# koadman/libMems

Measured on AMD Instinct MI355X. Metric: seed-mers/sec sorted+matched (+ MUMs/sec) at 1/2/4/8 MI355X; HBM GB/s vs roofline, higher is better.
Workload: dtype u64; 1 GPU; BASELINE config 3: 8 x 100 Mbp, seed weight 19 (0x7b974ef), MemHash seed stage (sorted+matched); genomes=8, genome_length=100000000, seedmers_total=799999792, seedmers_rank0=799999792, probes_rank0=100459493, parallelism=1 GPU

## Files before the change

include/mums.h:

```cpp
#ifndef MUMS_H
#define MUMS_H

#include <stdint.h>

#ifdef __cplusplus
extern "C" {
#endif

#define MUMS_ABI_VERSION 6

enum mums_status {
    MUMS_OK = 0,
    MUMS_E_INVALID = -1,
    MUMS_E_NOMEM = -2,
    MUMS_E_HIP = -3,
    MUMS_E_GAP = -4,
    MUMS_E_UNSUPPORTED = -5,
    MUMS_E_NODEVICE = -6
};

enum mums_stage {
    MUMS_STAGE_SEEDS = 1,
    MUMS_STAGE_ALL = 2
};
// ... 40 lines not shown

int  mums_set_seed(mums_ctx* ctx, uint64_t pattern);
int  mums_set_params(mums_ctx* ctx, uint32_t repeat_tol, uint32_t enum_tol, uint32_t table_size);
int  mums_set_mask(mums_ctx* ctx, int masked, uint64_t seq_mask);
int  mums_set_parallel_compat(mums_ctx* ctx, int enable, uint64_t chunk_size);
int  mums_set_pairwise(mums_ctx* ctx, int enable);

int  mums_add_genome(mums_ctx* ctx, const char* ascii, uint64_t n);
int  mums_add_genome_device(mums_ctx* ctx, const void* d_ascii, uint64_t n);
int  mums_genome_device(mums_ctx* ctx, uint32_t genome, const void** d_ascii, uint64_t* n);
int  mums_clear(mums_ctx* ctx);
int  mums_clear_sequences(mums_ctx* ctx);

int  mums_set_start_points(mums_ctx* ctx, const uint64_t* start_points, uint32_t count);
int  mums_get_offset_log(mums_ctx* ctx, uint64_t* out, uint64_t cap_rows, uint64_t* rows, uint32_t* seq_count);
int  mums_find(mums_ctx* ctx);
int  mums_find_stage(mums_ctx* ctx, int stage);

int  mums_result_count(mums_ctx* ctx, uint64_t* count, uint32_t* seq_count);
int  mums_result_copy(mums_ctx* ctx, uint64_t* lengths, int64_t* starts);

int  mums_mem_table_count(mums_ctx* ctx, uint32_t* counts, uint32_t table_size);
int  mums_get_stats(mums_ctx* ctx, mums_stats* out);
int  mums_set_profiling(mums_ctx* ctx, int enable);
const char* mums_last_error(mums_ctx* ctx);

int64_t  mums_get_seed(int weight, int seed_rank);
uint32_t mums_default_seed_weight(uint64_t avg_len);
int  mums_copy_seed_keys(mums_ctx* ctx, uint32_t genome, uint64_t* out, uint64_t cap);
int  mums_copy_seed_keys_range(mums_ctx* ctx, uint32_t genome, uint64_t first, uint64_t count, uint64_t* out);
int  mums_build_sml(mums_ctx* ctx, uint32_t genome, uint32_t* positions, uint64_t cap);
int  mums_seed_occurrence(mums_ctx* ctx, uint32_t genome, float* freq, uint64_t cap);
int  mums_multiplicity_filter(mums_ctx* ctx, uint32_t multiplicity);
int  mums_write_sml(mums_ctx* ctx, uint32_t genome, const char* path, const char* description);
int  mums_add_genome_sml(mums_ctx* ctx, const char* path, uint64_t* seed_out);
int  mums_length_filter(mums_ctx* ctx, uint64_t min_length);
int  mums_set_match_log(mums_ctx* ctx, int enable);
int  mums_match_log_copy(mums_ctx* ctx, uint64_t* lengths, int64_t* starts, uint64_t capacity, uint64_t* count);
int  mums_set_progress_log(mums_ctx* ctx, int enable);
int  mums_progress_log_copy(mums_ctx* ctx, char* text, uint64_t capacity, uint64_t* length);
int  mums_eliminate_overlaps(mums_ctx* ctx);
int  mums_eliminate_overlaps_v2(mums_ctx* ctx, const uint32_t* seq_ids, uint32_t count, int eliminate_both);
int  mums_load_matches(mums_ctx* ctx, uint32_t seq_count, uint64_t count, const uint64_t* lengths,
                       const int64_t* starts);
int  mums_find_batch(mums_ctx* ctx, uint32_t B, uint32_t G, const char* ascii, const uint64_t* seq_off);
int  mums_batch_info(mums_ctx* ctx, uint64_t* match_off, uint64_t* probes, uint64_t* collisions, uint64_t* restarts);
int  mums_anchor_batch(mums_ctx* ctx, uint32_t B, uint32_t G, const char* ascii, const uint64_t* seq_off,
                       const uint64_t* patterns, uint32_t rounds, int eliminate_both, uint64_t min_length);
int  mums_anchor_tail_batch(mums_ctx* ctx, uint32_t B, uint32_t G, const uint64_t* match_off,
                            const uint64_t* lengths, const int64_t* starts, int eliminate_both, uint64_t min_length);
int  mums_anchor_batch_info(mums_ctx* ctx, uint64_t* match_off, uint64_t* table_entries, uint64_t* probes,
                            uint64_t* collisions, uint64_t* restarts);
int  mums_debug_std_sort(mums_ctx* ctx, const uint64_t* keys, uint64_t n, int depth_override, uint32_t* ids);

int  mums_shard_layout(mums_ctx* ctx, uint32_t genomes_total, uint32_t first_genome, const uint64_t* lengths);
int  mums_shard_slice(mums_ctx* ctx, uint32_t genomes_total, const uint64_t* lengths, uint32_t genome,
                      uint64_t pos_begin, uint64_t pos_end);
int  mums_shard_msd_bits(mums_ctx* ctx, uint32_t* msd_bits, uint64_t* local_records);
int  mums_shard_keys(mums_ctx* ctx, uint64_t* d_records, uint64_t capacity, uint64_t* bucket_counts);
int  mums_shard_merge(mums_ctx* ctx, const uint64_t* d_records, uint32_t nsources, uint32_t first_bucket,
                      uint32_t nbuckets, const uint64_t* counts);
int  mums_shard_restart_pending(mums_ctx* ctx, uint64_t* pending);
int  mums_shard_stream(mums_ctx* ctx, const void** d_records, uint64_t* n);
int  mums_shard_restart_plan(mums_ctx* ctx, uint64_t* d_stream, uint32_t nranks, const uint64_t* counts,
                             const uint32_t* first_bucket, const uint32_t* nbuckets, void* d_out,
                             uint64_t capacity_bytes, uint64_t* block_bytes);
int  mums_shard_restart_apply(mums_ctx* ctx, const void* d_block, uint64_t restarts, const uint64_t* offset_log);
int  mums_shard_restart_counts(mums_ctx* ctx, uint64_t* info);
int  mums_shard_restart_prepare(mums_ctx* ctx, uint32_t nranks, uint32_t rank, const uint64_t* all_info,
                                uint64_t* S0);
int  mums_shard_restart_step(mums_ctx* ctx, uint64_t* S, uint64_t* restarts, uint64_t* undecidable);
int  mums_shard_restart_log(mums_ctx* ctx, uint64_t* rkey, uint64_t* rS);
int  mums_shard_restart_runs(mums_ctx* ctx, uint64_t restarts, const uint64_t* rkey, const uint64_t* rS,
                             uint64_t* runs, uint64_t capacity, uint64_t* nruns);
int  mums_shard_restart_ties(mums_ctx* ctx, const uint32_t* d_packed_all, const uint64_t* runs, uint64_t nruns,
                             const uint64_t* vofs, uint32_t* d_out);
int  mums_shard_restart_finish(mums_ctx* ctx, uint64_t restarts, const uint64_t* rkey, const uint64_t* rS,
                               const uint64_t* runs, uint64_t nruns, const uint32_t* d_pos, const uint64_t* vofs);
int  mums_shard_restart_info(mums_ctx* ctx, uint64_t* info);
int  mums_shard_tie_flags(mums_ctx* ctx, const uint64_t* gofs, uint32_t* d_out);
int  mums_shard_tie_replay(mums_ctx* ctx, const uint32_t* d_packed_all, uint32_t genome, uint32_t nparts,
                           const uint32_t* d_flags, const uint64_t* flag_off, const uint64_t* lens, uint32_t* d_out,
                           const uint64_t* out_off);
int  mums_shard_tie_apply(mums_ctx* ctx, const uint32_t* d_ids, const uint64_t* vofs);
int  mums_probe_count(mums_ctx* ctx, uint64_t* count);
int  mums_shard_bucket_counts(mums_ctx* ctx, uint64_t* counts);
int  mums_shard_probe_rows(mums_ctx* ctx, uint32_t nranks, const uint32_t* bounds, int64_t* d_rows,
                           uint64_t capacity_rows, uint64_t* counts);
int  mums_shard_packed_info(mums_ctx* ctx, uint64_t* word_offset, uint64_t* nwords, uint64_t* total_words);
int  mums_shard_packed_copy(mums_ctx* ctx, uint32_t* d_dst);
int  mums_shard_find(mums_ctx* ctx, const int64_t* d_rows, uint64_t nrows, const uint32_t* d_packed_all);
int  mums_shard_chain_label(mums_ctx* ctx, const uint32_t* d_packed_all, uint64_t* nchains);
int  mums_shard_chain_export(mums_ctx* ctx, uint32_t nranks, const uint32_t* bounds, int64_t* d_rows, uint32_t* d_tags,
                             uint64_t capacity_rows, int64_t* d_entries, uint32_t* d_first, uint64_t capacity_entries,
                             uint64_t* row_counts, uint64_t* entry_counts);
int  mums_shard_find_labelled(mums_ctx* ctx, const int64_t* d_rows, const uint32_t* d_tags, uint64_t nrows,
                              const int64_t* d_entries, const uint32_t* d_first, uint64_t nentries, uint32_t nsrc,
                              const uint64_t* src_rows, const uint64_t* src_entries, const uint32_t* d_packed_all);
int  mums_shard_chain_info(mums_ctx* ctx, uint64_t* info);
int  mums_shard_chain_entries(mums_ctx* ctx, uint32_t nranks, const uint32_t* bounds, int64_t* d_entries,
                              uint64_t capacity_entries, uint64_t* entry_counts);
int  mums_shard_entry_thresholds(mums_ctx* ctx, const int64_t* d_entries, uint64_t nentries, uint32_t* d_thr);
int  mums_shard_kept_export(mums_ctx* ctx, uint32_t nranks, const uint32_t* d_thr, int64_t* d_rows, uint32_t* d_tags,
                            uint64_t capacity_rows, uint32_t* d_first, uint64_t* row_counts, uint64_t* dropped_counts);
int  mums_shard_find_kept(mums_ctx* ctx, const int64_t* d_rows, const uint32_t* d_tags, uint64_t nrows,
                          const int64_t* d_entries, const uint32_t* d_first, uint64_t nentries, uint32_t nsrc,
// ... 29 lines not shown
```

libmems_amd/__init__.py:

```python
from __future__ import annotations

import ctypes
import os
from dataclasses import dataclass
from typing import List, Optional, Sequence

import numpy as np

_HERE = os.path.dirname(os.path.abspath(__file__))
LIB_PATH = os.environ.get("MUMS_DEV_LIB") or os.path.join(_HERE, "libmums_hip.so")

MUMS_OK = 0
MUMS_E_INVALID = -1
MUMS_E_NOMEM = -2
MUMS_E_HIP = -3
MUMS_E_GAP = -4
MUMS_E_UNSUPPORTED = -5
MUMS_E_NODEVICE = -6

STAGE_SEEDS = 1
STAGE_ALL = 2

DEFAULT_MEM_TABLE_SIZE = 40000
DEFAULT_REPEAT_TOLERANCE = 0
# ... 20 lines not shown
        ("mem_count", ctypes.c_uint64),
        ("collision_count", ctypes.c_uint64),
        ("repeat_limit_groups", ctypes.c_uint64),
        ("nonempty_buckets", ctypes.c_uint64),
        ("ms_keys", ctypes.c_double),
        ("ms_sort", ctypes.c_double),
        ("ms_groups", ctypes.c_double),
        ("ms_buckets", ctypes.c_double),
        ("ms_replay", ctypes.c_double),
        ("ms_output", ctypes.c_double),
        ("ms_total", ctypes.c_double),
        ("ms_dominant", ctypes.c_double),
        ("dominant_launches", ctypes.c_uint64),
        ("dominant_bytes", ctypes.c_uint64),
        ("key_bytes", ctypes.c_uint64),
        ("sort_passes", ctypes.c_uint64),
        ("ms_chains", ctypes.c_double),
        ("chains", ctypes.c_uint64),
        ("chunks", ctypes.c_uint64),
        ("restarts", ctypes.c_uint64),
        ("ms_chain_walks", ctypes.c_double),
        ("chain_walk_words", ctypes.c_uint64),
        ("chain_walks", ctypes.c_uint64),
        ("chain_walk_bytes", ctypes.c_uint64),
        ("ms_short_walks", ctypes.c_double),
        ("short_walk_words", ctypes.c_uint64),
        ("short_walks", ctypes.c_uint64),
        ("short_walk_bytes", ctypes.c_uint64),
    ]


EXPORTED_SYMBOLS = [
    "mums_abi_version", "mums_ctx_create", "mums_ctx_destroy", "mums_set_stream", "mums_set_seed",
    "mums_set_params", "mums_set_mask", "mums_add_genome", "mums_add_genome_device", "mums_clear",
    "mums_find", "mums_find_stage", "mums_result_count", "mums_result_copy", "mums_get_stats",
    "mums_last_error", "mums_get_seed", "mums_default_seed_weight", "mums_copy_seed_keys",
    "mums_build_sml", "mums_set_profiling", "mums_shard_layout", "mums_shard_msd_bits", "mums_shard_keys",
    "mums_shard_merge", "mums_probe_count", "mums_probe_copy", "mums_shard_bucket_counts", "mums_shard_probe_rows",
    "mums_shard_packed_info", "mums_shard_packed_copy", "mums_shard_find", "mums_set_parallel_compat",
    "mums_seed_occurrence", "mums_multiplicity_filter", "mums_length_filter", "mums_write_sml",
    "mums_add_genome_sml", "mums_set_pairwise", "mums_shard_slice", "mums_set_start_points",
    "mums_get_offset_log", "mums_copy_seed_keys_range", "mums_mem_table_count", "mums_eliminate_overlaps",
    "mums_load_matches", "mums_debug_std_sort", "mums_comm_unique_id", "mums_comm_init_rank", "mums_comm_init_all",
    "mums_comm_init_local", "mums_comm_destroy", "mums_comm_last_error", "mums_shard_key_ranges", "mums_shard_run",
    "mums_set_match_log", "mums_match_log_copy", "mums_shard_restart_pending", "mums_shard_stream",
    "mums_shard_restart_plan", "mums_shard_restart_apply", "mums_comm_init_host", "mums_set_progress_log",
    "mums_progress_log_copy", "mums_shard_restart_counts", "mums_shard_restart_prepare", "mums_shard_restart_step",
    "mums_shard_restart_log", "mums_shard_restart_runs", "mums_shard_restart_ties", "mums_shard_restart_finish",
    "mums_shard_restart_info", "mums_shard_tie_flags", "mums_shard_tie_replay", "mums_shard_tie_apply",
    "mums_genome_device", "mums_shard_chain_label", "mums_shard_chain_export", "mums_shard_find_labelled",
    "mums_shard_chain_info", "mums_shard_chain_entries", "mums_shard_entry_thresholds", "mums_shard_kept_export",
    "mums_shard_find_kept", "mums_comm_exchange_info", "mums_eliminate_overlaps_v2", "mums_clear_sequences",
    "mums_find_batch", "mums_batch_info", "mums_anchor_batch", "mums_anchor_tail_batch", "mums_anchor_batch_info",
]

COMM_ALLGATHER_FN = ctypes.CFUNCTYPE(ctypes.c_int, ctypes.c_void_p, ctypes.POINTER(ctypes.c_uint64), ctypes.c_uint64,
                                     ctypes.POINTER(ctypes.c_uint64))
COMM_ALLTOALLV_FN = ctypes.CFUNCTYPE(ctypes.c_int, ctypes.c_void_p, ctypes.c_void_p, ctypes.POINTER(ctypes.c_uint64),
                                     ctypes.c_void_p, ctypes.POINTER(ctypes.c_uint64))


class MumsCommOps(ctypes.Structure):
    _fields_ = [("allgather_u64", COMM_ALLGATHER_FN), ("alltoallv", COMM_ALLTOALLV_FN)]

_lib: Optional[ctypes.CDLL] = None


def load_library(path: str = LIB_PATH) -> ctypes.CDLL:
    global _lib
    if _lib is not None:
        return _lib
    if not os.path.exists(path):
        raise ImportError(f"{path} not built: run `make -C {_HERE}` (hipcc --offload-arch=gfx950)")
    try:
        import torch
    except ImportError:
        pass
    lib = ctypes.CDLL(path)
    vp, u64, u32, i32 = ctypes.c_void_p, ctypes.c_uint64, ctypes.c_uint32, ctypes.c_int
    lib.mums_abi_version.restype = i32
    lib.mums_ctx_create.argtypes = [i32, ctypes.POINTER(vp)]
    lib.mums_ctx_destroy.argtypes = [vp]
    lib.mums_set_stream.argtypes = [vp, vp]
    lib.mums_set_seed.argtypes = [vp, u64]
    lib.mums_set_params.argtypes = [vp, u32, u32, u32]
    lib.mums_set_mask.argtypes = [vp, i32, u64]
    lib.mums_add_genome.argtypes = [vp, ctypes.c_char_p, u64]
    lib.mums_add_genome_device.argtypes = [vp, vp, u64]
    lib.mums_genome_device.argtypes = [vp, u32, ctypes.POINTER(vp), ctypes.POINTER(u64)]
    lib.mums_shard_chain_label.argtypes = [vp, vp, vp]
    lib.mums_shard_chain_export.argtypes = [vp, u32, vp, vp, vp, u64, vp, vp, u64, vp, vp]
    lib.mums_shard_find_labelled.argtypes = [vp, vp, vp, u64, vp, vp, u64, u32, vp, vp, vp]
    lib.mums_shard_chain_info.argtypes = [vp, vp]
    lib.mums_shard_chain_entries.argtypes = [vp, u32, vp, vp, u64, vp]
    lib.mums_shard_entry_thresholds.argtypes = [vp, vp, u64, vp]
    lib.mums_shard_kept_export.argtypes = [vp, u32, vp, vp, vp, u64, vp, vp, vp]
    lib.mums_shard_find_kept.argtypes = [vp, vp, vp, u64, vp, vp, u64, u32, vp, vp, u64, vp]
    lib.mums_comm_exchange_info.argtypes = [vp, vp]
    lib.mums_clear.argtypes = [vp]
    lib.mums_clear_sequences.argtypes = [vp]
    lib.mums_find.argtypes = [vp]
    lib.mums_find_stage.argtypes = [vp, i32]
    lib.mums_result_count.argtypes = [vp, ctypes.POINTER(u64), ctypes.POINTER(u32)]
    lib.mums_result_copy.argtypes = [vp, vp, vp]
    lib.mums_get_stats.argtypes = [vp, ctypes.POINTER(_Stats)]
    lib.mums_last_error.argtypes = [vp]
    lib.mums_last_error.restype = ctypes.c_char_p
    lib.mums_get_seed.argtypes = [i32, i32]
    lib.mums_get_seed.restype = ctypes.c_int64
    lib.mums_default_seed_weight.argtypes = [u64]
    lib.mums_default_seed_weight.restype = u32
    lib.mums_copy_seed_keys.argtypes = [vp, u32, vp, u64]
    lib.mums_build_sml.argtypes = [vp, u32, vp, u64]
    lib.mums_set_profiling.argtypes = [vp, i32]
    lib.mums_shard_layout.argtypes = [vp, u32, u32, vp]
    lib.mums_shard_msd_bits.argtypes = [vp, ctypes.POINTER(u32), ctypes.POINTER(u64)]
    lib.mums_shard_keys.argtypes = [vp, vp, u64, vp]
    lib.mums_shard_merge.argtypes = [vp, vp, u32, u32, u32, vp]
    lib.mums_probe_count.argtypes = [vp, ctypes.POINTER(u64)]
    lib.mums_probe_copy.argtypes = [vp, vp, vp, u64]
    lib.mums_shard_bucket_counts.argtypes = [vp, vp]
    lib.mums_shard_probe_rows.argtypes = [vp, u32, vp, vp, u64, vp]
    lib.mums_shard_packed_info.argtypes = [vp, ctypes.POINTER(u64), ctypes.POINTER(u64), ctypes.POINTER(u64)]
    lib.mums_shard_packed_copy.argtypes = [vp, vp]
    lib.mums_shard_find.argtypes = [vp, vp, u64, vp]
    lib.mums_set_parallel_compat.argtypes = [vp, i32, u64]
    lib.mums_seed_occurrence.argtypes = [vp, u32, vp, u64]
    lib.mums_multiplicity_filter.argtypes = [vp, u32]
    lib.mums_length_filter.argtypes = [vp, u64]
    lib.mums_write_sml.argtypes = [vp, u32, ctypes.c_char_p, ctypes.c_char_p]
    lib.mums_add_genome_sml.argtypes = [vp, ctypes.c_char_p, ctypes.POINTER(u64)]
    lib.mums_set_pairwise.argtypes = [vp, i32]
    lib.mums_shard_slice.argtypes = [vp, u32, vp, u32, u64, u64]
    lib.mums_set_start_points.argtypes = [vp, vp, u32]
    lib.mums_copy_seed_keys_range.argtypes = [vp, u32, u64, u64, vp]
    lib.mums_mem_table_count.argtypes = [vp, vp, u32]
    lib.mums_get_offset_log.argtypes = [vp, vp, u64, ctypes.POINTER(u64), ctypes.POINTER(u32)]
    lib.mums_eliminate_overlaps.argtypes = [vp]
    lib.mums_eliminate_overlaps_v2.argtypes = [vp, vp, u32, ctypes.c_int]
    lib.mums_load_matches.argtypes = [vp, u32, u64, vp, vp]
    lib.mums_debug_std_sort.argtypes = [vp, vp, u64, ctypes.c_int, vp]
    lib.mums_comm_unique_id.argtypes = [vp, u64]
    lib.mums_comm_init_rank.argtypes = [ctypes.POINTER(vp), ctypes.c_int, ctypes.c_int, ctypes.c_int, vp]
    lib.mums_comm_init_all.argtypes = [ctypes.POINTER(vp), ctypes.c_int, vp]
    lib.mums_comm_init_local.argtypes = [ctypes.POINTER(vp), ctypes.c_int, vp]
    lib.mums_comm_init_host.argtypes = [ctypes.POINTER(vp), ctypes.c_int, ctypes.c_int, ctypes.c_int,
                                        ctypes.POINTER(MumsCommOps), vp]
    lib.mums_comm_destroy.argtypes = [vp]
    lib.mums_comm_destroy.restype = None
    lib.mums_comm_last_error.argtypes = [vp]
    lib.mums_comm_last_error.restype = ctypes.c_char_p
    lib.mums_shard_key_ranges.argtypes = [vp, u32, u32, vp, vp]
    lib.mums_shard_run.argtypes = [vp, vp, ctypes.c_int]
    lib.mums_shard_restart_pending.argtypes = [vp, vp]
    lib.mums_shard_stream.argtypes = [vp, vp, vp]
    lib.mums_shard_restart_plan.argtypes = [vp, vp, u32, vp, vp, vp, vp, u64, vp]
    lib.mums_shard_restart_apply.argtypes = [vp, vp, u64, vp]
    lib.mums_shard_restart_counts.argtypes = [vp, vp]
    lib.mums_shard_restart_prepare.argtypes = [vp, u32, u32, vp, vp]
    lib.mums_shard_restart_step.argtypes = [vp, vp, vp, vp]
    lib.mums_shard_restart_log.argtypes = [vp, vp, vp]
    lib.mums_shard_restart_runs.argtypes = [vp, u64, vp, vp, vp, u64, vp]
    lib.mums_shard_restart_ties.argtypes = [vp, vp, vp, u64, vp, vp]
    lib.mums_shard_restart_finish.argtypes = [vp, u64, vp, vp, vp, u64, vp, vp]
    lib.mums_shard_restart_info.argtypes = [vp, vp]
    lib.mums_shard_tie_flags.argtypes = [vp, vp, vp]
    lib.mums_shard_tie_replay.argtypes = [vp, vp, u32, u32, vp, vp, vp, vp, vp]
    lib.mums_shard_tie_apply.argtypes = [vp, vp, vp]
    lib.mums_set_match_log.argtypes = [vp, i32]
    lib.mums_set_progress_log.argtypes = [vp, i32]
    lib.mums_progress_log_copy.argtypes = [vp, ctypes.c_char_p, u64, ctypes.POINTER(u64)]
    lib.mums_match_log_copy.argtypes = [vp, vp, vp, u64, ctypes.POINTER(u64)]
    lib.mums_find_batch.argtypes = [vp, u32, u32, vp, vp]
    lib.mums_batch_info.argtypes = [vp, vp, vp, vp, vp]
    lib.mums_anchor_batch.argtypes = [vp, u32, u32, vp, vp, vp, u32, i32, u64]
    lib.mums_anchor_tail_batch.argtypes = [vp, u32, u32, vp, vp, vp, i32, u64]
    lib.mums_anchor_batch_info.argtypes = [vp, vp, vp, vp, vp, vp]
    _lib = lib
    return lib


def getSeed(weight: int, seed_rank: int = 0) -> int:
    return int(load_library().mums_get_seed(weight, seed_rank)) & 0xFFFFFFFFFFFFFFFF


def getSeedLength(seed: int) -> int:
    if seed == 0:
        return 0
    s = seed & 0xFFFFFFFFFFFFFFFF
    lo = (s & -s).bit_length() - 1
    return s.bit_length() - lo


def getSeedWeight(seed: int) -> int:
# ... 384 lines not shown

    def SetMatchLog(self, enable: bool = True) -> None:
        self._check(self._lib.mums_set_match_log(self._ctx, int(bool(enable))))

    def MatchLog(self) -> "MatchList":
        n = ctypes.c_uint64()
        self._check(self._lib.mums_match_log_copy(self._ctx, None, None, 0, ctypes.byref(n)))
        g = ctypes.c_uint32()
        cnt = ctypes.c_uint64()
        self._check(self._lib.mums_result_count(self._ctx, ctypes.byref(cnt), ctypes.byref(g)))
        lengths = np.zeros(n.value, dtype=np.uint64)
        starts = np.zeros((n.value, g.value), dtype=np.int64)
        if n.value:
            self._check(self._lib.mums_match_log_copy(self._ctx, lengths.ctypes.data, starts.ctypes.data, n.value,
                                                      ctypes.byref(n)))
        return MatchList(lengths, starts)

    def LogProgress(self, enable: bool = True) -> None:
        self._check(self._lib.mums_set_progress_log(self._ctx, int(bool(enable))))

    def ProgressLog(self) -> str:
        n = ctypes.c_uint64()
        self._check(self._lib.mums_progress_log_copy(self._ctx, None, 0, ctypes.byref(n)))
        buf = ctypes.create_string_buffer(n.value + 1)
        self._check(self._lib.mums_progress_log_copy(self._ctx, buf, n.value + 1, ctypes.byref(n)))
        return buf.value.decode()

    def EliminateOverlaps(self) -> None:
        self._check(self._lib.mums_eliminate_overlaps(self._ctx))

    def EliminateOverlaps_v2(self, seq_ids=None, eliminate_both: bool = False) -> None:
        if seq_ids is None:
            self._check(self._lib.mums_eliminate_overlaps_v2(self._ctx, None, 0, int(bool(eliminate_both))))
            return
        for i in seq_ids:
            if not 0 <= int(i) < 2 ** 32:
                raise MumsError(MUMS_E_INVALID, f"EliminateOverlaps_v2: sequence id {i} out of range")
        n = len(seq_ids)
        ids = np.zeros(max(n, 1), dtype=np.uint32)
        ids[:n] = [int(i) for i in seq_ids]
        self._check(self._lib.mums_eliminate_overlaps_v2(self._ctx, ids.ctypes.data, n, int(bool(eliminate_both))))

    def LoadMatches(self, ml: "MatchList") -> None:
        lengths = np.ascontiguousarray(ml.lengths, dtype=np.uint64)
        starts = np.ascontiguousarray(ml.starts, dtype=np.int64)
        M, G = starts.shape
        self._check(self._lib.mums_load_matches(self._ctx, G, M, lengths.ctypes.data, starts.ctypes.data))

    def _debug_std_sort(self, keys: np.ndarray, depth: int = -1) -> np.ndarray:
        keys = np.ascontiguousarray(keys, dtype=np.uint64)
        ids = np.zeros(len(keys), dtype=np.uint32)
        self._check(self._lib.mums_debug_std_sort(self._ctx, keys.ctypes.data, len(keys), depth, ids.ctypes.data))
        return ids


def shard_key_ranges(totals, world: int):
    lib = load_library()
    t = np.ascontiguousarray(totals, dtype=np.uint64)
    f = np.zeros(world, dtype=np.uint32)
    c = np.zeros(world, dtype=np.uint32)
    rc = lib.mums_shard_key_ranges(t.ctypes.data, len(t), world, f.ctypes.data, c.ctypes.data)
    if rc != MUMS_OK:
        raise MumsError(rc, "mums_shard_key_ranges")
    return [(int(a), int(b)) for a, b in zip(f, c)]


class ShardedMemHash:

    def __init__(self, devices: Sequence[int], comm: str = "rccl", table_size: int = 40000, layout: str = "blocks",
                 parallel_compat: bool = False, chunk_size: int = 200000, pairwise: bool = False):
        if layout not in ("blocks", "slices"):
            raise ValueError("layout: 'blocks' or 'slices'")
        self.layout = layout
        self.parallel_compat = bool(parallel_compat)
        self.pairwise = bool(pairwise)
        self.chunk_size = int(chunk_size)
        self._lib = load_library()
        self.devices = list(devices)
        self.world = len(self.devices)
        self.comm_kind = comm
        self.table_size = table_size
        self.seed = 0
        self.repeat_tol = 0
        self.enum_tol = 1
        self.progress = False
        self.match_log = False
        self.seqs: List[bytes] = []
        self.ranks: List[MemHash] = []
        self.stats_per_rank: List[dict] = []
        self.rank_status: List[int] = []
        comms = (ctypes.c_void_p * self.world)()
        devs = (ctypes.c_int * self.world)(*self.devices)
        init = self._lib.mums_comm_init_all if comm == "rccl" else self._lib.mums_comm_init_local
        rc = init(comms, self.world, devs)
        if rc != MUMS_OK:
            raise MumsError(rc, f"mums_comm_init ({comm}) failed")
        self._comms = [comms[r] for r in range(self.world)]

    def SetSeed(self, seed: int) -> None:
        self.seed = seed

    def SetRepeatTolerance(self, t: int) -> None:
        self.repeat_tol = int(t)

    def SetEnumerationTolerance(self, t: int) -> None:
        self.enum_tol = int(t)
# ... 189 lines not shown
```

libmems_amd/csrc/mums_capi.hip:

```cpp
#include <hip/hip_runtime.h>

#include <algorithm>
#include <array>
#include <chrono>
#include <functional>
#include <cstddef>
#include <cstdio>
#include <cstdlib>
#include <cstring>
#include <memory>
#include <string>
#include <vector>

#include "../../include/mums.h"
#include "match_device.h"
#include "mums_internal.h"
#include "seed_device.h"

using namespace mums;

namespace {

struct DevBuf {
    void* p = nullptr;
// ... 3699 lines not shown
    }
    uint64_t P = 0, C = 0, R = 0, E = 0;
    for (uint32_t p = 0; p < B; ++p) {
        P += ctx->batch_probes[p];
        C += ctx->batch_coll[p];
        R += ctx->batch_restarts[p];
        E += ctx->anchor_table[p];
    }
    mums_stats& s = ctx->st;
    s = mums_stats{};
    s.seedmers = Nstat;
    s.probes = P;
    s.mem_count = E;
    s.collision_count = C;
    s.restarts = R;
    s.repeat_limit_groups = R;
    s.key_bytes = 8;
    for (const Round& x : rd) s.sort_passes += (uint64_t)((x.kbits + pbits + 7) / 8);
    s.ms_keys = ms_keys;
    s.ms_sort = ms_sort;
    s.ms_replay = ms_replay;
    s.ms_output = anchor_ms(ctx, EV_REPLAY, EV_OUTPUT);
    s.ms_total = anchor_ms(ctx, EV_START, EV_OUTPUT);
    return anchor_done(ctx, G, M, P, Nstat);
}

int mums_anchor_batch_info(mums_ctx* ctx, uint64_t* match_off, uint64_t* table_entries, uint64_t* probes,
                           uint64_t* collisions, uint64_t* restarts) {
    if (check_ctx(ctx)) return MUMS_E_INVALID;
    if (!ctx->batch_result || !ctx->anchor_result)
        return fail(ctx, MUMS_E_INVALID, "no completed mums_anchor_batch / mums_anchor_tail_batch on this context");
    if (match_off) std::copy(ctx->batch_off.begin(), ctx->batch_off.end(), match_off);
    if (table_entries) std::copy(ctx->anchor_table.begin(), ctx->anchor_table.end(), table_entries);
    if (probes) std::copy(ctx->batch_probes.begin(), ctx->batch_probes.end(), probes);
    if (collisions) std::copy(ctx->batch_coll.begin(), ctx->batch_coll.end(), collisions);
    if (restarts) std::copy(ctx->batch_restarts.begin(), ctx->batch_restarts.end(), restarts);
    return MUMS_OK;
}

int mums_debug_std_sort(mums_ctx* ctx, const uint64_t* keys, uint64_t n, int depth_override, uint32_t* ids) {
    if (check_ctx(ctx) || (n && (!keys || !ids))) return MUMS_E_INVALID;
    if (n >= 0xFFFFFFF0ull) return fail(ctx, MUMS_E_UNSUPPORTED, "n >= 2^32");
    if (n == 0) return MUMS_OK;
    HIPCHK(hipSetDevice(ctx->device));
    HIPCHK(ctx->flen.ensure(n * 8 + 8));
    HIPCHK(ctx->fs.ensure(n * 4 + 8));
    HIPCHK(h2d_sync(ctx->flen.p, keys, n * 8, ctx->stream));
    HIPCHK(eo_sort_ids(ctx->eo, ctx->flen.as<uint64_t>(), (uint32_t)n, depth_override, ctx->fs.as<uint32_t>(),
                       ctx->stream));
    HIPCHK(hipMemcpy(ids, ctx->fs.p, n * 4, hipMemcpyDeviceToHost));
    return MUMS_OK;
}


int mums_shard_layout(mums_ctx* ctx, uint32_t genomes_total, uint32_t first_genome, const uint64_t* lengths) {
    if (check_ctx(ctx)) return MUMS_E_INVALID;
    if (genomes_total > (uint32_t)kMaxG) return fail(ctx, MUMS_E_UNSUPPORTED, "more than 64 genomes");
    if (first_genome > genomes_total || (genomes_total && !lengths))
        return fail(ctx, MUMS_E_INVALID, "bad shard layout");
    ctx->shard = true;
    ctx->slice = false;
    ctx->shard_first = first_genome;
    ctx->shard_len.assign(lengths, lengths + genomes_total);
    ctx->stage_done = 0;
    return MUMS_OK;
}

int mums_shard_slice(mums_ctx* ctx, uint32_t genomes_total, const uint64_t* lengths, uint32_t genome,
                     uint64_t pos_begin, uint64_t pos_end) {
    if (check_ctx(ctx)) return MUMS_E_INVALID;
    if (genomes_total > (uint32_t)kMaxG) return fail(ctx, MUMS_E_UNSUPPORTED, "more than 64 genomes");
    if (genome >= genomes_total || !lengths || pos_begin > pos_end) return fail(ctx, MUMS_E_INVALID, "bad slice");
    ctx->shard = true;
    ctx->slice = true;
    ctx->shard_first = genome;
    ctx->slice_genome = genome;
    ctx->slice_begin = pos_begin;
    ctx->slice_end = pos_end;
    ctx->shard_len.assign(lengths, lengths + genomes_total);
    ctx->stage_done = 0;
    return MUMS_OK;
}

int mums_shard_msd_bits(mums_ctx* ctx, uint32_t* msd_bits, uint64_t* local_records) {
    if (check_ctx(ctx)) return MUMS_E_INVALID;
    int rc = prepare_shard(ctx);
    if (rc) return rc;
    if (msd_bits) *msd_bits = (uint32_t)ctx->msd_bits;
    if (local_records) {
        uint64_t n = 0;
        for (int g = 0; g < ctx->lgt.G; ++g) n += ctx->lgt.m[g];
        *local_records = n;
    }
    return MUMS_OK;
}

int mums_shard_keys(mums_ctx* ctx, uint64_t* d_records, uint64_t capacity, uint64_t* bucket_counts) {
    if (check_ctx(ctx)) return MUMS_E_INVALID;
    if (!have_device()) return fail(ctx, MUMS_E_NODEVICE, "no HIP device");
    HIPCHK(hipSetDevice(ctx->device));
    int rc = prepare_shard(ctx);
    if (rc) return rc;
    GenomeTable& l = ctx->lgt;
    uint64_t n = 0;
    for (int g = 0; g < l.G; ++g) n += l.m[g];
    if (n > capacity || (n && !d_records)) return fail(ctx, MUMS_E_INVALID, "record buffer too small");
// ... 2704 lines not shown
```

libmems_amd/csrc/radix_sort.hip:

```cpp
#include <cstdlib>
#include "mums_internal.h"

namespace mums {

namespace {

constexpr int kRTile = 4096;
constexpr int kRounds = kRTile / kBlock;
constexpr int kWaves = kBlock / 64;
constexpr int kDigits = 256;

template <typename K>
__global__ __launch_bounds__(kBlock) void rs_upsweep(const K* __restrict__ keys, uint64_t n, int shift,
                                                     uint32_t* __restrict__ hist, uint32_t nblocks, int agg) {
    __shared__ uint32_t h[kWaves][kDigits];
    const int lane = threadIdx.x & 63, wv = threadIdx.x >> 6;
    for (int i = threadIdx.x; i < kWaves * kDigits; i += kBlock) (&h[0][0])[i] = 0;
    __syncthreads();
    const uint64_t b0 = (uint64_t)blockIdx.x * kRTile + (uint64_t)wv * (kRTile / kWaves);
    if (agg) {
        #pragma unroll 4
        for (int r = 0; r < kRounds; ++r) {
            const uint64_t i = b0 + (uint64_t)r * 64 + lane;
            const bool valid = i < n;
            const uint32_t d = valid ? (uint32_t)(keys[i] >> shift) & 0xFFu : 0u;
            uint32_t tot;
            const uint32_t rk = wave_match_rank<8>(d, valid, &tot);
            if (valid && rk == 0) atomicAdd(&h[wv][d], tot);
        }
    } else {
        #pragma unroll 4
        for (int r = 0; r < kRounds; ++r) {
            uint64_t i = b0 + (uint64_t)r * 64 + lane;
            if (i < n) {
                uint32_t d = (uint32_t)(keys[i] >> shift) & 0xFFu;
                atomicAdd(&h[wv][d], 1u);
            }
        }
    }
    __syncthreads();
    const int t = threadIdx.x;
    uint32_t s = 0;
    #pragma unroll
    for (int w = 0; w < kWaves; ++w) s += h[w][t];
    hist[(uint64_t)t * nblocks + blockIdx.x] = s;
}

template <typename K, bool kImplicitVals>
__global__ __launch_bounds__(kBlock) void rs_downsweep(const K* __restrict__ kin, const uint32_t* __restrict__ vin,
                                                       uint64_t n, int shift, const uint32_t* __restrict__ hist,
                                                       uint32_t nblocks, K* __restrict__ kout,
                                                       uint32_t* __restrict__ vout) {
    __shared__ K skeys[kRTile];
    __shared__ uint32_t svals[kRTile];
    __shared__ uint32_t wcnt[kWaves][kDigits];
    __shared__ uint32_t lstart[kDigits];
    __shared__ uint32_t gofs[kDigits];
    __shared__ uint32_t s_w[kWaves];
    const int lane = threadIdx.x & 63, wv = threadIdx.x >> 6;
    for (int i = threadIdx.x; i < kWaves * kDigits; i += kBlock) (&wcnt[0][0])[i] = 0;
    __syncthreads();

    const uint64_t tile0 = (uint64_t)blockIdx.x * kRTile;
    const uint64_t b0 = tile0 + (uint64_t)wv * (kRTile / kWaves);
    K key[kRounds];
    uint32_t val[kRounds];
    uint32_t rank[kRounds];
    #pragma unroll
    for (int r = 0; r < kRounds; ++r) {
        const uint64_t i = b0 + (uint64_t)r * 64 + lane;
        const bool valid = i < n;
        key[r] = valid ? kin[i] : (K)0;
        val[r] = kImplicitVals ? (uint32_t)i : (valid ? vin[i] : 0u);
        const uint32_t d = (uint32_t)(key[r] >> shift) & 0xFFu;
        uint32_t tot;
        const uint32_t rk = wave_match_rank<8>(d, valid, &tot);
        uint32_t old = 0;
        if (valid) old = wcnt[wv][d];
        if (valid && rk == 0) wcnt[wv][d] = old + tot;
        rank[r] = old + rk;
    }
    __syncthreads();

    {
        const int t = threadIdx.x;
        uint32_t acc = 0;
        #pragma unroll
        for (int w = 0; w < kWaves; ++w) {
            uint32_t c = wcnt[w][t];
            wcnt[w][t] = acc;
            acc += c;
        }
        uint32_t v = acc;
        #pragma unroll
        for (int d = 1; d < 64; d <<= 1) {
            uint32_t x = __shfl_up(v, d, 64);
            if (lane >= d) v += x;
        }
        if (lane == 63) s_w[wv] = v;
        __syncthreads();
        uint32_t wpre = 0;
        #pragma unroll
        for (int w = 0; w < kWaves; ++w) wpre += (w < wv) ? s_w[w] : 0u;
        lstart[t] = wpre + v - acc;
        gofs[t] = hist[(uint64_t)t * nblocks + blockIdx.x];
    }
    __syncthreads();

    #pragma unroll
    for (int r = 0; r < kRounds; ++r) {
        const uint64_t i = b0 + (uint64_t)r * 64 + lane;
        if (i < n) {
            const uint32_t d = (uint32_t)(key[r] >> shift) & 0xFFu;
            const uint32_t lp = lstart[d] + wcnt[wv][d] + rank[r];
            skeys[lp] = key[r];
            svals[lp] = val[r];
        }
    }
    __syncthreads();

    const uint64_t cnt = (n - tile0) < (uint64_t)kRTile ? (n - tile0) : (uint64_t)kRTile;
    #pragma unroll
    for (int r = 0; r < kRounds; ++r) {
        const uint32_t s = threadIdx.x + r * kBlock;
        if (s < cnt) {
            const K k = skeys[s];
            const uint32_t d = (uint32_t)(k >> shift) & 0xFFu;
            const uint64_t o = (uint64_t)gofs[d] + (s - lstart[d]);
            kout[o] = k;
            vout[o] = svals[s];
        }
    }
}

uint64_t tiles(uint64_t n) { return (n + kRTile - 1) / kRTile; }

}

size_t radix_tmp_bytes(uint64_t n) {
    uint64_t h = (uint64_t)kDigits * tiles(n);
    return (h + 64) * sizeof(uint32_t) + scan_tmp_bytes(h) + 256;
}

template <typename K>
hipError_t radix_sort(const K* keys_in, const uint32_t* vals_in, uint64_t n, int bits, K* kA, uint32_t* vA,
                      K* kB, uint32_t* vB, void* d_tmp, int* out_buf, hipStream_t st, hipEvent_t* ev_ds) {
    const int passes = (bits + 7) / 8;
    *out_buf = (passes - 1) % 2;
    if (n == 0 || passes == 0) return hipSuccess;
    const uint32_t nb = (uint32_t)tiles(n);
    uint32_t* hist = (uint32_t*)d_tmp;
    void* stmp = (void*)(hist + (uint64_t)kDigits * nb + 64);
    const K* ksrc = keys_in;
    const uint32_t* vsrc = vals_in;
    for (int p = 0; p < passes; ++p) {
        K* kdst = (p % 2 == 0) ? kA : kB;
        uint32_t* vdst = (p % 2 == 0) ? vA : vB;
        const int shift = 8 * p;
        const bool agg = !getenv("MUMS_DEV_RS_NOAGG");
        hipLaunchKernelGGL(rs_upsweep<K>, dim3(nb), dim3(kBlock), 0, st, ksrc, n, shift, hist, nb, agg ? 1 : 0);
        hipError_t e = exclusive_scan_u32(hist, (uint64_t)kDigits * nb, stmp, nullptr, st);
        if (e != hipSuccess) return e;
        if (ev_ds) (void)hipEventRecord(ev_ds[2 * p], st);
        if (vsrc == nullptr)
            hipLaunchKernelGGL((rs_downsweep<K, true>), dim3(nb), dim3(kBlock), 0, st, ksrc, vsrc, n, shift, hist,
                               nb, kdst, vdst);
        else
            hipLaunchKernelGGL((rs_downsweep<K, false>), dim3(nb), dim3(kBlock), 0, st, ksrc, vsrc, n, shift, hist,
                               nb, kdst, vdst);
        e = hipGetLastError();
        if (e != hipSuccess) return e;
        if (ev_ds) (void)hipEventRecord(ev_ds[2 * p + 1], st);
        ksrc = kdst;
        vsrc = vdst;
    }
    return hipSuccess;
}

template hipError_t radix_sort<uint32_t>(const uint32_t*, const uint32_t*, uint64_t, int, uint32_t*, uint32_t*,
                                         uint32_t*, uint32_t*, void*, int*, hipStream_t, hipEvent_t*);
template hipError_t radix_sort<uint64_t>(const uint64_t*, const uint32_t*, uint64_t, int, uint64_t*, uint32_t*,
                                         uint64_t*, uint32_t*, void*, int*, hipStream_t, hipEvent_t*);

}
```

Before: 40.03 billion seed-mers/s.

## Restructure radix sort upsweep and specialize downsweep on digit width

Rewrites the radix upsweep so that each wave counts a whole 4096-key tile using vectorized 16-byte loads and ballot-based digit aggregation. Each block now covers several tiles and writes the histograms out in coalesced order. The downsweep is templated on the actual digit bit-width of the last pass and runs with 512 threads, using 16-bit per-wave counters. These changes target memory throughput and shared-memory atomic cost in the sort. They add complexity and more template instantiations, and the uint16 counters could overflow if the tile size grows. A debug entry point for timing the radix sort is also added.

```diff
diff --git a/include/mums.h b/include/mums.h
--- a/include/mums.h
+++ b/include/mums.h
@@ -116,6 +116,8 @@
 int  mums_anchor_batch_info(mums_ctx* ctx, uint64_t* match_off, uint64_t* table_entries, uint64_t* probes,
                             uint64_t* collisions, uint64_t* restarts);
 int  mums_debug_std_sort(mums_ctx* ctx, const uint64_t* keys, uint64_t n, int depth_override, uint32_t* ids);
+int  mums_debug_radix_sort(mums_ctx* ctx, const void* d_keys, int key_bytes, uint64_t n, int bits,
+                           void* d_keys_out, uint32_t* d_ids_out, float* ms);
 
 int  mums_shard_layout(mums_ctx* ctx, uint32_t genomes_total, uint32_t first_genome, const uint64_t* lengths);
 int  mums_shard_slice(mums_ctx* ctx, uint32_t genomes_total, const uint64_t* lengths, uint32_t genome,
diff --git a/libmems_amd/__init__.py b/libmems_amd/__init__.py
--- a/libmems_amd/__init__.py
+++ b/libmems_amd/__init__.py
@@ -96,6 +96,7 @@
     "mums_shard_chain_info", "mums_shard_chain_entries", "mums_shard_entry_thresholds", "mums_shard_kept_export",
     "mums_shard_find_kept", "mums_comm_exchange_info", "mums_eliminate_overlaps_v2", "mums_clear_sequences",
     "mums_find_batch", "mums_batch_info", "mums_anchor_batch", "mums_anchor_tail_batch", "mums_anchor_batch_info",
+    "mums_debug_radix_sort",
 ]
 
 COMM_ALLGATHER_FN = ctypes.CFUNCTYPE(ctypes.c_int, ctypes.c_void_p, ctypes.POINTER(ctypes.c_uint64), ctypes.c_uint64,
@@ -184,6 +185,7 @@
     lib.mums_eliminate_overlaps_v2.argtypes = [vp, vp, u32, ctypes.c_int]
     lib.mums_load_matches.argtypes = [vp, u32, u64, vp, vp]
     lib.mums_debug_std_sort.argtypes = [vp, vp, u64, ctypes.c_int, vp]
+    lib.mums_debug_radix_sort.argtypes = [vp, vp, i32, u64, i32, vp, vp, ctypes.POINTER(ctypes.c_float)]
     lib.mums_comm_unique_id.argtypes = [vp, u64]
     lib.mums_comm_init_rank.argtypes = [ctypes.POINTER(vp), ctypes.c_int, ctypes.c_int, ctypes.c_int, vp]
     lib.mums_comm_init_all.argtypes = [ctypes.POINTER(vp), ctypes.c_int, vp]
@@ -674,6 +676,20 @@
         ids = np.zeros(len(keys), dtype=np.uint32)
         self._check(self._lib.mums_debug_std_sort(self._ctx, keys.ctypes.data, len(keys), depth, ids.ctypes.data))
         return ids
+
+    def _debug_radix_sort(self, keys, bits: int):
+        import torch
+
+        if keys.dim() != 1 or not keys.is_cuda or not keys.is_contiguous() or keys.element_size() not in (4, 8):
+            raise MumsError(MUMS_E_INVALID, "_debug_radix_sort: a contiguous 1-D device tensor of 4-B or 8-B keys")
+        n = keys.numel()
+        kout = torch.empty_like(keys)
+        ids = torch.empty(n, dtype=torch.int32, device=keys.device)
+        ms = ctypes.c_float(0.0)
+        torch.cuda.synchronize(keys.device)
+        self._check(self._lib.mums_debug_radix_sort(self._ctx, keys.data_ptr(), keys.element_size(), n, int(bits),
+                                                    kout.data_ptr(), ids.data_ptr(), ctypes.byref(ms)))
+        return kout, ids, float(ms.value)
 
 
 def shard_key_ranges(totals, world: int):
diff --git a/libmems_amd/csrc/mums_capi.hip b/libmems_amd/csrc/mums_capi.hip
--- a/libmems_amd/csrc/mums_capi.hip
+++ b/libmems_amd/csrc/mums_capi.hip
@@ -3775,6 +3775,49 @@
     return MUMS_OK;
 }
 
+int mums_debug_radix_sort(mums_ctx* ctx, const void* d_keys, int key_bytes, uint64_t n, int bits, void* d_keys_out,
+                          uint32_t* d_ids_out, float* ms) {
+    if (check_ctx(ctx) || (n && (!d_keys || !d_keys_out || !d_ids_out))) return MUMS_E_INVALID;
+    if ((key_bytes != 4 && key_bytes != 8) || bits < 1 || bits > 8 * key_bytes)
+        return fail(ctx, MUMS_E_INVALID, "mums_debug_radix_sort: key_bytes 4 or 8, 1 <= bits <= 8 * key_bytes");
+    if (n >= 0xFFFFFFF0ull) return fail(ctx, MUMS_E_UNSUPPORTED, "n >= 2^32");
+    if (ms) *ms = 0.f;
+    if (n == 0) return MUMS_OK;
+    HIPCHK(hipSetDevice(ctx->device));
+    HIPCHK(ctx->flen.ensure(n * (size_t)key_bytes + 8));
+    HIPCHK(ctx->fs.ensure(n * 4 + 8));
+    HIPCHK(ctx->radix_tmp.ensure(radix_tmp_bytes(n + 1)));
+    hipStream_t st = ctx->stream;
+    struct Ev {
+        hipEvent_t e[2] = {nullptr, nullptr};
+        ~Ev() {
+            for (hipEvent_t x : e)
+                if (x) (void)hipEventDestroy(x);
+        }
+    } ev;
+    HIPCHK(hipEventCreate(&ev.e[0]));
+    HIPCHK(hipEventCreate(&ev.e[1]));
+    const bool out_is_a = (((bits + 7) / 8 - 1) % 2) == 0;
+    void* ko = ctx->flen.p;
+    uint32_t* io = ctx->fs.as<uint32_t>();
+    int out = 0;
+    HIPCHK(hipEventRecord(ev.e[0], st));
+    if (key_bytes == 8)
+        HIPCHK(radix_sort<uint64_t>((const uint64_t*)d_keys, nullptr, n, bits,
+                                    (uint64_t*)(out_is_a ? d_keys_out : ko), out_is_a ? d_ids_out : io,
+                                    (uint64_t*)(out_is_a ? ko : d_keys_out), out_is_a ? io : d_ids_out,
+                                    ctx->radix_tmp.p, &out, st));
+    else
+        HIPCHK(radix_sort<uint32_t>((const uint32_t*)d_keys, nullptr, n, bits,
+                                    (uint32_t*)(out_is_a ? d_keys_out : ko), out_is_a ? d_ids_out : io,
+                                    (uint32_t*)(out_is_a ? ko : d_keys_out), out_is_a ? io : d_ids_out,
+                                    ctx->radix_tmp.p, &out, st));
+    HIPCHK(hipEventRecord(ev.e[1], st));
+    HIPCHK(hipStreamSynchronize(st));
+    if (ms) HIPCHK(hipEventElapsedTime(ms, ev.e[0], ev.e[1]));
+    return MUMS_OK;
+}
+
 
 int mums_shard_layout(mums_ctx* ctx, uint32_t genomes_total, uint32_t first_genome, const uint64_t* lengths) {
     if (check_ctx(ctx)) return MUMS_E_INVALID;
diff --git a/libmems_amd/csrc/radix_sort.hip b/libmems_amd/csrc/radix_sort.hip
--- a/libmems_amd/csrc/radix_sort.hip
+++ b/libmems_amd/csrc/radix_sort.hip
@@ -6,36 +6,113 @@
 namespace {
 
 constexpr int kRTile = 4096;
-constexpr int kRounds = kRTile / kBlock;
 constexpr int kWaves = kBlock / 64;
 constexpr int kDigits = 256;
 
+constexpr int kUpTiles = 16;
+constexpr uint32_t kUpFew = 2048;
+constexpr uint32_t kUpMany = 8192;
+constexpr int kUpPad = kUpTiles + 1;
+
+__device__ __forceinline__ void count_round(uint32_t* h, uint32_t d, bool valid, int lane, bool agg) {
+    if (!agg) {
+        if (valid) atomicAdd(&h[d], 1u);
+        return;
+    }
+    const uint64_t rem = __ballot(valid);
+    const uint32_t m = (uint32_t)__builtin_amdgcn_readlane((int)d, rem ? __builtin_ctzll(rem) : 0);
+    const bool hit = valid && d == m;
+    const uint64_t eq = __ballot(hit);
+    if (lane == 0) h[m] += (uint32_t)__builtin_popcountll(eq);
+    __builtin_amdgcn_wave_barrier();
+    const bool left = valid && !hit;
+    const uint64_t lm = __ballot(left);
+    if (lm) {
+        uint32_t tot;
+        const uint32_t rk = wave_match_rank_from<8>(d, (uint32_t)lm, (uint32_t)(lm >> 32), &tot);
+        if (left && rk == 0) h[d] += tot;
+    }
+    __builtin_amdgcn_wave_barrier();
+}
+
 template <typename K>
 __global__ __launch_bounds__(kBlock) void rs_upsweep(const K* __restrict__ keys, uint64_t n, int shift,
-                                                     uint32_t* __restrict__ hist, uint32_t nblocks, int agg) {
+                                                     uint32_t dmask, uint32_t* __restrict__ hist, uint32_t nblocks,
+                                                     int agg, int tsh) {
+    constexpr int kV = 16 / (int)sizeof(K);
+    constexpr int kLoads = kRTile / (64 * kV);
+    struct alignas(16) Vec { K k[kV]; };
+    __shared__ uint32_t cnt[kDigits * kUpPad];
+    __shared__ uint32_t h[kWaves][kDigits];
+    const int lane = threadIdx.x & 63, wv = threadIdx.x >> 6;
+    uint32_t* hw = h[wv];
+    #pragma unroll
+    for (int q = 0; q < kDigits / 64; ++q) hw[q * 64 + lane] = 0;
+    const uint32_t tpb = 1u << tsh, nwaves = blockDim.x >> 6;
+    const uint32_t t0 = blockIdx.x << tsh;
+    const uint32_t nt = (nblocks - t0) < tpb ? (nblocks - t0) : tpb;
+    const bool aligned = (reinterpret_cast<uintptr_t>(keys) & 15u) == 0;
+    for (uint32_t j = wv; j < nt; j += nwaves) {
+        const uint64_t b0 = (uint64_t)(t0 + j) * kRTile;
+        if (aligned && b0 + kRTile <= n) {
+            #pragma unroll 1
+            for (int q0 = 0; q0 < kLoads; q0 += 4) {
+                Vec v[4];
+                #pragma unroll
+                for (int q = 0; q < 4; ++q)
+                    v[q] = *reinterpret_cast<const Vec*>(keys + b0 + (uint64_t)(q0 + q) * (64 * kV) +
+                                                         (uint64_t)lane * kV);
+                #pragma unroll
+                for (int q = 0; q < 4; ++q) {
+                    #pragma unroll
+                    for (int e = 0; e < kV; ++e)
+                        count_round(hw, (uint32_t)(v[q].k[e] >> shift) & dmask, true, lane, agg != 0);
+                }
+            }
+        } else {
+            #pragma unroll 4
+            for (int r = 0; r < kRTile / 64; ++r) {
+                const uint64_t i = b0 + (uint64_t)r * 64 + lane;
+                const bool valid = i < n;
+                const uint32_t d = valid ? (uint32_t)(keys[i] >> shift) & dmask : 0u;
+                count_round(hw, d, valid, lane, agg != 0);
+            }
+        }
+        #pragma unroll
+        for (int q = 0; q < kDigits / 64; ++q) {
+            const int d = q * 64 + lane;
+            cnt[d * kUpPad + j] = hw[d];
+            hw[d] = 0;
+        }
+    }
+    __syncthreads();
+    for (uint32_t i = threadIdx.x; i < ((uint32_t)kDigits << tsh); i += blockDim.x) {
+        const uint32_t d = i >> tsh, j = i & (tpb - 1);
+        if (j < nt) hist[(uint64_t)d * nblocks + t0 + j] = cnt[d * kUpPad + j];
+    }
+}
+
+template <typename K>
+__global__ __launch_bounds__(kBlock) void rs_upsweep_tile(const K* __restrict__ keys, uint64_t n, int shift,
+                                                          uint32_t dmask, uint32_t* __restrict__ hist,
+                                                          uint32_t nblocks, int agg) {
+    constexpr int kRounds = kRTile / kBlock;
     __shared__ uint32_t h[kWaves][kDigits];
     const int lane = threadIdx.x & 63, wv = threadIdx.x >> 6;
     for (int i = threadIdx.x; i < kWaves * kDigits; i += kBlock) (&h[0][0])[i] = 0;
     __syncthreads();
     const uint64_t b0 = (uint64_t)blockIdx.x * kRTile + (uint64_t)wv * (kRTile / kWaves);
-    if (agg) {
-        #pragma unroll 4
-        for (int r = 0; r < kRounds; ++r) {
-            const uint64_t i = b0 + (uint64_t)r * 64 + lane;
-            const bool valid = i < n;
-            const uint32_t d = valid ? (uint32_t)(keys[i] >> shift) & 0xFFu : 0u;
+    #pragma unroll 4
+    for (int r = 0; r < kRounds; ++r) {
+        const uint64_t i = b0 + (uint64_t)r * 64 + lane;
+        const bool valid = i < n;
+        const uint32_t d = valid ? (uint32_t)(keys[i] >> shift) & dmask : 0u;
+        if (agg) {
             uint32_t tot;
             const uint32_t rk = wave_match_rank<8>(d, valid, &tot);
             if (valid && rk == 0) atomicAdd(&h[wv][d], tot);
-        }
-    } else {
-        #pragma unroll 4
-        for (int r = 0; r < kRounds; ++r) {
-            uint64_t i = b0 + (uint64_t)r * 64 + lane;
-            if (i < n) {
-                uint32_t d = (uint32_t)(keys[i] >> shift) & 0xFFu;
-                atomicAdd(&h[wv][d], 1u);
-            }
+        } else if (valid) {
+            atomicAdd(&h[wv][d], 1u);
         }
     }
     __syncthreads();
@@ -46,72 +123,80 @@
     hist[(uint64_t)t * nblocks + blockIdx.x] = s;
 }
 
-template <typename K, bool kImplicitVals>
-__global__ __launch_bounds__(kBlock) void rs_downsweep(const K* __restrict__ kin, const uint32_t* __restrict__ vin,
-                                                       uint64_t n, int shift, const uint32_t* __restrict__ hist,
-                                                       uint32_t nblocks, K* __restrict__ kout,
-                                                       uint32_t* __restrict__ vout) {
+template <typename K, bool kImplicitVals, int kRB, int kT>
+__global__ __launch_bounds__(kT) void rs_downsweep(const K* __restrict__ kin, const uint32_t* __restrict__ vin,
+                                                         uint64_t n, int shift, const uint32_t* __restrict__ hist,
+                                                         uint32_t nblocks, K* __restrict__ kout,
+                                                         uint32_t* __restrict__ vout) {
     __shared__ K skeys[kRTile];
     __shared__ uint32_t svals[kRTile];
-    __shared__ uint32_t wcnt[kWaves][kDigits];
+    __shared__ alignas(16) uint16_t wcnt[kT / 64][kDigits];
     __shared__ uint32_t lstart[kDigits];
     __shared__ uint32_t gofs[kDigits];
-    __shared__ uint32_t s_w[kWaves];
+    __shared__ uint32_t s_w[kDigits / 64];
+    constexpr uint32_t kDMask = (1u << kRB) - 1u;
+    constexpr int kDsBlock = kT, kDsWaves = kT / 64, kDsRounds = kRTile / kT;
     const int lane = threadIdx.x & 63, wv = threadIdx.x >> 6;
-    for (int i = threadIdx.x; i < kWaves * kDigits; i += kBlock) (&wcnt[0][0])[i] = 0;
-    __syncthreads();
-
-    const uint64_t tile0 = (uint64_t)blockIdx.x * kRTile;
-    const uint64_t b0 = tile0 + (uint64_t)wv * (kRTile / kWaves);
-    K key[kRounds];
-    uint32_t val[kRounds];
-    uint32_t rank[kRounds];
-    #pragma unroll
-    for (int r = 0; r < kRounds; ++r) {
+    const int t = threadIdx.x;
+    for (int i = threadIdx.x; i < kDsWaves * kDigits / 2; i += kDsBlock) ((uint32_t*)&wcnt[0][0])[i] = 0;
+
+    const uint32_t tile = blockIdx.x;
+    uint32_t gpre = 0;
+    if (t < kDigits) gpre = hist[(uint64_t)t * nblocks + tile];
+    __syncthreads();
+
+    const uint64_t tile0 = (uint64_t)tile * kRTile;
+    const uint64_t b0 = tile0 + (uint64_t)wv * (kRTile / kDsWaves);
+    K key[kDsRounds];
+    uint32_t val[kDsRounds];
+    uint32_t rank[kDsRounds];
+    #pragma unroll
+    for (int r = 0; r < kDsRounds; ++r) {
         const uint64_t i = b0 + (uint64_t)r * 64 + lane;
         const bool valid = i < n;
         key[r] = valid ? kin[i] : (K)0;
         val[r] = kImplicitVals ? (uint32_t)i : (valid ? vin[i] : 0u);
-        const uint32_t d = (uint32_t)(key[r] >> shift) & 0xFFu;
+        const uint32_t d = (uint32_t)(key[r] >> shift) & kDMask;
         uint32_t tot;
-        const uint32_t rk = wave_match_rank<8>(d, valid, &tot);
+        const uint32_t rk = wave_match_rank<kRB>(d, valid, &tot);
         uint32_t old = 0;
         if (valid) old = wcnt[wv][d];
-        if (valid && rk == 0) wcnt[wv][d] = old + tot;
+        if (valid && rk == 0) wcnt[wv][d] = (uint16_t)(old + tot);
         rank[r] = old + rk;
     }
     __syncthreads();
 
-    {
-        const int t = threadIdx.x;
-        uint32_t acc = 0;
+    uint32_t acc = 0, v = 0;
+    if (t < kDigits) {
         #pragma unroll
-        for (int w = 0; w < kWaves; ++w) {
+        for (int w = 0; w < kDsWaves; ++w) {
             uint32_t c = wcnt[w][t];
-            wcnt[w][t] = acc;
+            wcnt[w][t] = (uint16_t)acc;
             acc += c;
         }
-        uint32_t v = acc;
+        v = acc;
         #pragma unroll
         for (int d = 1; d < 64; d <<= 1) {
             uint32_t x = __shfl_up(v, d, 64);
             if (lane >= d) v += x;
         }
         if (lane == 63) s_w[wv] = v;
-        __syncthreads();
+    }
+    __syncthreads();
+    if (t < kDigits) {
         uint32_t wpre = 0;
         #pragma unroll
-        for (int w = 0; w < kWaves; ++w) wpre += (w < wv) ? s_w[w] : 0u;
+        for (int w = 0; w < kDigits / 64; ++w) wpre += (w < wv) ? s_w[w] : 0u;
         lstart[t] = wpre + v - acc;
-        gofs[t] = hist[(uint64_t)t * nblocks + blockIdx.x];
-    }
-    __syncthreads();
-
-    #pragma unroll
-    for (int r = 0; r < kRounds; ++r) {
+        gofs[t] = gpre;
+    }
+    __syncthreads();
+
+    #pragma unroll
+    for (int r = 0; r < kDsRounds; ++r) {
         const uint64_t i = b0 + (uint64_t)r * 64 + lane;
         if (i < n) {
-            const uint32_t d = (uint32_t)(key[r] >> shift) & 0xFFu;
+            const uint32_t d = (uint32_t)(key[r] >> shift) & kDMask;
             const uint32_t lp = lstart[d] + wcnt[wv][d] + rank[r];
             skeys[lp] = key[r];
             svals[lp] = val[r];
@@ -121,11 +206,11 @@
 
     const uint64_t cnt = (n - tile0) < (uint64_t)kRTile ? (n - tile0) : (uint64_t)kRTile;
     #pragma unroll
-    for (int r = 0; r < kRounds; ++r) {
-        const uint32_t s = threadIdx.x + r * kBlock;
+    for (int r = 0; r < kDsRounds; ++r) {
+        const uint32_t s = threadIdx.x + r * kDsBlock;
         if (s < cnt) {
             const K k = skeys[s];
-            const uint32_t d = (uint32_t)(k >> shift) & 0xFFu;
+            const uint32_t d = (uint32_t)(k >> shift) & kDMask;
             const uint64_t o = (uint64_t)gofs[d] + (s - lstart[d]);
             kout[o] = k;
             vout[o] = svals[s];
@@ -134,6 +219,33 @@
 }
 
 uint64_t tiles(uint64_t n) { return (n + kRTile - 1) / kRTile; }
+
+template <typename K, int kRB>
+void launch_downsweep_rb(const K* kin, const uint32_t* vin, uint64_t n, int shift, const uint32_t* hist, uint32_t nb,
+                         K* kout, uint32_t* vout, hipStream_t st) {
+    constexpr int kT = 512;
+    if (vin == nullptr)
+        hipLaunchKernelGGL((rs_downsweep<K, true, kRB, kT>), dim3(nb), dim3(kT), 0, st, kin, vin, n, shift, hist, nb,
+                           kout, vout);
+    else
+        hipLaunchKernelGGL((rs_downsweep<K, false, kRB, kT>), dim3(nb), dim3(kT), 0, st, kin, vin, n, shift, hist, nb,
+                           kout, vout);
+}
+
+template <typename K>
+void launch_downsweep(int rb, const K* kin, const uint32_t* vin, uint64_t n, int shift, const uint32_t* hist,
+                      uint32_t nb, K* kout, uint32_t* vout, hipStream_t st) {
+    switch (rb) {
+        case 1: return launch_downsweep_rb<K, 1>(kin, vin, n, shift, hist, nb, kout, vout, st);
+        case 2: return launch_downsweep_rb<K, 2>(kin, vin, n, shift, hist, nb, kout, vout, st);
+        case 3: return launch_downsweep_rb<K, 3>(kin, vin, n, shift, hist, nb, kout, vout, st);
+        case 4: return launch_downsweep_rb<K, 4>(kin, vin, n, shift, hist, nb, kout, vout, st);
+        case 5: return launch_downsweep_rb<K, 5>(kin, vin, n, shift, hist, nb, kout, vout, st);
+        case 6: return launch_downsweep_rb<K, 6>(kin, vin, n, shift, hist, nb, kout, vout, st);
+        case 7: return launch_downsweep_rb<K, 7>(kin, vin, n, shift, hist, nb, kout, vout, st);
+        default: return launch_downsweep_rb<K, 8>(kin, vin, n, shift, hist, nb, kout, vout, st);
+    }
+}
 
 }
 
@@ -158,16 +270,19 @@
         uint32_t* vdst = (p % 2 == 0) ? vA : vB;
         const int shift = 8 * p;
         const bool agg = !getenv("MUMS_DEV_RS_NOAGG");
-        hipLaunchKernelGGL(rs_upsweep<K>, dim3(nb), dim3(kBlock), 0, st, ksrc, n, shift, hist, nb, agg ? 1 : 0);
+        const int rb = (bits - shift) < 8 ? (bits - shift) : 8;
+        if (nb < kUpFew) {
+            hipLaunchKernelGGL(rs_upsweep_tile<K>, dim3(nb), dim3(kBlock), 0, st, ksrc, n, shift, (1u << rb) - 1u, hist,
+                               nb, agg ? 1 : 0);
+        } else {
+            const int tsh = nb >= kUpMany ? 4 : 2;
+            hipLaunchKernelGGL(rs_upsweep<K>, dim3((nb + (1u << tsh) - 1) >> tsh), dim3(kBlock), 0, st, ksrc, n, shift,
+                               (1u << rb) - 1u, hist, nb, agg ? 1 : 0, tsh);
+        }
         hipError_t e = exclusive_scan_u32(hist, (uint64_t)kDigits * nb, stmp, nullptr, st);
         if (e != hipSuccess) return e;
         if (ev_ds) (void)hipEventRecord(ev_ds[2 * p], st);
-        if (vsrc == nullptr)
-            hipLaunchKernelGGL((rs_downsweep<K, true>), dim3(nb), dim3(kBlock), 0, st, ksrc, vsrc, n, shift, hist,
-                               nb, kdst, vdst);
-        else
-            hipLaunchKernelGGL((rs_downsweep<K, false>), dim3(nb), dim3(kBlock), 0, st, ksrc, vsrc, n, shift, hist,
-                               nb, kdst, vdst);
+        launch_downsweep<K>(rb, ksrc, vsrc, n, shift, hist, nb, kdst, vdst, st);
         e = hipGetLastError();
         if (e != hipSuccess) return e;
         if (ev_ds) (void)hipEventRecord(ev_ds[2 * p + 1], st);
```

Measured after the change: 40.43 billion seed-mers/s, median of 5. No clear change (+1.0%).
